# blyssprivacy/sdk

Measured on NVIDIA H100. Metric: PIR server queries/sec (Spiral process_query), higher is better.
Workload: dtype u64

## Files before the change

sdk_b200/csrc/api.cu:

```cuda
#include "../../include/b200pir.h"
#include "kernels.h"
#include "ntt_tables.hpp"
#include <cstdio>
#include <algorithm>
#include <cmath>
#include <memory>
#include <cstring>
#include <condition_variable>
#include <chrono>
#include <deque>
#include <mutex>
#include <set>
#include <string>
#include <utility>
#include <vector>

using namespace b200pir;

namespace b200pir {
thread_local unsigned long long g_kernel_launches = 0;

void opt_in_smem_impl(const void* kernel, int bytes) {
  static std::mutex mu;
  static std::set<std::pair<const void*, int>> done;
// ... 49 lines not shown
  int device = 0;
  cudaStream_t stream = nullptr;
  bool own_stream = true;
  std::recursive_mutex mu;
  b200pir_params hp;
  int dim0, num_per, slices, trials, g, stop_round, num_packing;
  int bits_gsw, bits_conv, bits_left, bits_right;
  bool has_right;
  uint64_t q2, q1, setup_bytes, query_bytes, response_bytes;
  int q1_bits;
  DevParams dp;
  DevBuf<Twiddle> d_tw;
  DevBuf<Twiddle> d_tw4k;
  DevBuf<uint32_t> d_neg1;
  int mul_variant = 0, max_group = 16, profile = 0;
  int fold_variant = 2;
  int intt_variant = 0;
  int expand_variant = 0;
  long pair_min_ctas = 528;
  int sparse_fold = 0;
  int imma_variant = 0;
  int db_format = -1;
  DevBuf<uint2> w_qf;
  DevBuf<uint8_t> w_qt;
  int sm_count = 0;
  size_t ws_queries = 0, ws_rows = 0;
  DevBuf<uint64_t> w_query;
  DevBuf<uint32_t> w_v;
  DevBuf<uint32_t> w_zflags;
  DevBuf<uint32_t> w_xr;
  DevBuf<uint4> w_qdev;
  DevBuf<uint32_t> w_vfold, w_vfold_neg;
  DevBuf<uint32_t> w_mult;
  DevBuf<uint32_t> w_cts;
// ... 258 lines not shown
}

const uint32_t* run_fold_res(b200pir_ctx* c, uint32_t* a, uint32_t* b, size_t batch, size_t batch_stride, size_t num,
                             int k0, const uint32_t* vfold, int slices_per_query) {
  const size_t mat = (size_t)2 * 2 * c->hp.t_gsw * 2 * POLY;
  int k = k0;
  uint32_t* src = a;
  uint32_t* dst = b;
  uint32_t* zero_flags = nullptr;
  if (c->sparse_fold) {
    c->w_zflags.ensure(batch * num);
    zero_flags = c->w_zflags.p;
  }
  for (size_t half = num / 2; half >= 1; half /= 2, k--) {
    launch_fold_res(c->dp, src, dst, batch, batch_stride, (int)half, vfold + (size_t)k * mat, c->fold_words(),
                    slices_per_query, (int)c->hp.t_gsw, c->bits_gsw, c->fold_variant, zero_flags, c->stream);
    std::swap(src, dst);
  }
  return src;
}

void run_prepare(b200pir_ctx* c, b200pir_pp* pp, size_t count, bool images = false) {
  b200pir_ctx::Scope sc(c, ST_EXPAND);
  if (images) c->w_qt.ensure((count + 15) / 16 * tc5_query_bytes(make_tc5_geom(c->dim0, 32)));
  if (c->hp.expand_queries)
    run_expand_query(c, pp, c->w_query.p, c->w_v.p, c->w_qdev.p, c->w_vfold.p, (int)count, images ? c->w_qt.p : nullptr);
}

void run_first_dim_and_fold(b200pir_ctx* c, b200pir_db* db, size_t count, const uint4* qdev = nullptr,
                            const uint32_t* vfold = nullptr, const uint8_t* images = nullptr, size_t per_group = 16) {
  if (!qdev) qdev = c->w_qdev.p;
// ... 241 lines not shown
  if (queries == 0 || queries > 4096 || rows_local == 0 || rows_local > ((size_t)1 << c->hp.nu_2))
    throw Error(B200PIR_E_BADARG, "reserve: 1..4096 queries, 1..num_per rows");
  Guard gd(c);
  B200_CUDA(cudaStreamSynchronize(c->stream));
  c->ensure_workspace(queries, rows_local);
  B200_CUDA(cudaGetLastError());
  API_END
}
int b200pir_ctx_set_option(b200pir_ctx* c, const char* key, int64_t value) {
  API_BEGIN
  if (!c || !key) throw Error(B200PIR_E_BADARG, "null argument");
  Guard gd(c);
  std::string k(key);
  if (k == "mul_variant") c->mul_variant = (int)value;
  else if (k == "batch") { if (value != 1 && value != 2 && value != 4 && value != 8 && value != 16) throw Error(B200PIR_E_BADARG, "batch must be 1, 2, 4, 8 or 16"); c->max_group = (int)value; }
  else if (k == "fold_variant") c->fold_variant = (int)value;
  else if (k == "intt_variant") c->intt_variant = (int)value;
  else if (k == "imma_variant") c->imma_variant = (int)value;
  else if (k == "sparse_fold") c->sparse_fold = value != 0;
  else if (k == "coalesce") c->coalesce = value != 0;
  else if (k == "coalesce_window_us") { if (value < 0 || value > 100000) throw Error(B200PIR_E_BADARG, "coalesce_window_us must be 0..100000"); c->coalesce_window_us = (int)value; }
  else if (k == "expand_variant") c->expand_variant = (int)value;
  else if (k == "expand_pair_min_ctas") c->pair_min_ctas = (long)value;
  else if (k == "db_format") { if (value < -1 || value > 2) throw Error(B200PIR_E_BADARG, "db_format must be -1 (automatic), 0, 1 or 2"); c->db_format = (int)value; }
  else if (k == "profile") {
    if (value < 0 || value > 2) throw Error(B200PIR_E_BADARG, "profile must be 0, 1 or 2");
    c->profile = (int)value;
    c->spans.clear(); c->event_next = 0; c->mul_launches = 0;
  }
  else throw Error(B200PIR_E_BADARG, "unknown option " + k);
  API_END
// ... 526 lines not shown
  B200_CUDA(cudaMemcpyAsync(wide.p, v_folding, wide.n * 8, cudaMemcpyHostToDevice, c->stream));
  launch_narrow(vf.p, wide.p, wide.n, c->stream);
  if (v_folding_neg && !c->sparse_fold) {
    DevBuf<uint32_t> vfn(c->fold_words());
    B200_CUDA(cudaMemcpyAsync(wide.p, v_folding_neg, wide.n * 8, cudaMemcpyHostToDevice, c->stream));
    launch_narrow(vfn.p, wide.p, wide.n, c->stream);
    run_fold(c, cts.p, 1, num * 2 * POLY, num, dims - 1, vf.p, vfn.p, 1);
  } else {
    DevBuf<uint32_t> a(num * 4 * POLY), b(num * 4 * POLY);
    DevBuf<uint32_t> zflags;
    if (c->sparse_fold) zflags.alloc(num);
    launch_raw_to_res(c->dp, a.p, cts.p, num * 2, c->stream);
    int k = dims - 1;
    for (size_t half = num / 2; half >= 1; half /= 2, k--) {
      launch_fold_res(c->dp, a.p, b.p, 1, num * 4 * POLY, (int)half, vf.p + (size_t)k * mat, c->fold_words(), 1,
                      (int)c->hp.t_gsw, c->bits_gsw, c->fold_variant, zflags.p, c->stream);
      B200_CUDA(cudaMemcpyAsync(a.p, b.p, half * 4 * POLY * 4, cudaMemcpyDeviceToDevice, c->stream));
    }
    launch_res_to_raw(c->dp, cts.p, a.p, num * 2, c->stream);
  }
  B200_CUDA(cudaMemcpyAsync(v_cts, cts.p, cts.n * 8, cudaMemcpyDeviceToHost, c->stream));
  B200_CUDA(cudaStreamSynchronize(c->stream));
  B200_CUDA(cudaGetLastError());
  API_END
}

int b200pir_get_v_folding_neg(b200pir_ctx* c, uint64_t* out, const uint64_t* v_folding) {
  API_BEGIN
  if (!c || !out || !v_folding) throw Error(B200PIR_E_BADARG, "null argument");
  Guard gd(c);
  const size_t words = c->fold_words();
// ... 696 lines not shown
```

sdk_b200/csrc/kernels.h:

```cpp
#pragma once
#include "common.cuh"
#include "tc5_layout.cuh"

namespace b200pir {

static const int POLY = 2048;

extern thread_local unsigned long long g_kernel_launches;

void opt_in_smem_impl(const void* kernel, int bytes);
template <typename K>
inline void opt_in_smem(K* kernel, int bytes) { opt_in_smem_impl(reinterpret_cast<const void*>(kernel), bytes); }

void launch_ntt_u64(const DevParams& P, uint64_t* polys, size_t count, bool inverse, cudaStream_t s);
void launch_ntt32(const DevParams& P, uint32_t* polys, size_t count, bool inverse, cudaStream_t s);
void launch_ntt32_4k(uint32_t q0, uint32_t q1, const Twiddle* tw, uint32_t* polys, size_t count, bool inverse, cudaStream_t s);
void launch_to_ntt(const DevParams& P, uint32_t* out, const uint64_t* raw, size_t count, cudaStream_t s);
void launch_to_ntt_strided(const DevParams& P, uint32_t* out, size_t out_stride, const uint64_t* raw, size_t raw_stride,
                           size_t count, int batches, cudaStream_t s);
void launch_chacha_first_rows(uint64_t* raw, const uint8_t seed[32], uint64_t word0, uint32_t n_mats, uint32_t row_words,
                              uint64_t mat_words, uint64_t modulus, cudaStream_t s);
void launch_direct_query_to_dev(uint4* q_dev, const uint32_t* sig_ntt, const uint64_t* wire_words, int dim0, cudaStream_t s);
void launch_from_ntt(const DevParams& P, uint64_t* out_raw, const uint32_t* in, size_t count, cudaStream_t s);
void launch_raw_to_res(const DevParams& P, uint32_t* out, const uint64_t* raw, size_t polys, cudaStream_t s);
// ... 36 lines not shown
size_t tc5_db_bytes(const Tc5Geom& T, int slices);
size_t tc5_query_bytes(const Tc5Geom& T);
bool tc5_supported(const Tc5Geom& T);
void launch_db_to_tc5(const Tc5Geom& T, const uint4* db0_slice, uint8_t* dbt, int slice, cudaStream_t s);
void launch_db_upsert_tc5(const Tc5Geom& T, uint8_t* dbt, int slice, int il, int j, const uint64_t* poly, cudaStream_t s);
void launch_query_to_tc5(const Tc5Geom& T, const uint4* q_dev, size_t q_stride, int nq, uint8_t* qt, cudaStream_t s);
void launch_reorient_to_tc5(const Tc5Geom& T, const uint32_t* v, size_t v_stride, int idx_factor, int nq, uint8_t* qt, cudaStream_t s);
void launch_multiply_tc5(const DevParams& P, const Tc5Geom& T, const uint8_t* dbt, const uint32_t* tile_mask, const uint8_t* qt,
                         uint32_t* out_zm, size_t out_stride, int nq, int slice_begin, int slice_count, int sm_count, cudaStream_t s);

void launch_fold_round(const DevParams& P, uint64_t* cts, size_t batch, size_t batch_stride , int half,
                       const uint32_t* c_pos, const uint32_t* c_neg, size_t c_batch_stride ,
                       int slices_per_query, int t_gsw, int bits, cudaStream_t s);
void launch_fold_res(const DevParams& P, const uint32_t* in, uint32_t* out, size_t batch, size_t batch_stride ,
                     int half, const uint32_t* c_pos, size_t c_batch_stride, int slices_per_query, int t_gsw, int bits,
                     int variant, uint32_t* zero_flags , cudaStream_t s);
void launch_folding_neg(const DevParams& P, uint32_t* out, const uint32_t* v_folding, int count, int t_gsw, int bits,
                        cudaStream_t s);

void launch_expand_scalar(const DevParams& P, uint32_t* v, size_t v_stride, int nq, int num_in, const uint32_t* neg1_r,
                          cudaStream_t s);
struct PpTable { const uint32_t* const* pack; const uint32_t* const* left; const uint32_t* const* right; const uint32_t* const* conv; };
struct ExpandRound {
  int r, num_in, stop_round, max_bits_to_gen_right, t_auto;
  const uint32_t* const* tab_left;
  const uint32_t* const* tab_right;
  size_t off_left, off_right;
  int t_left, t_right, bits_left, bits_right;
  int fill_skipped;
};
void launch_expand_round(const DevParams& P, uint32_t* v, size_t v_stride, int nq, const ExpandRound& R, cudaStream_t s);
// ... 32 lines not shown
```

sdk_b200/csrc/poly_kernels.cu:

```cuda
#include "kernels.h"
#include "ntt_core4096.cuh"

namespace b200pir {

namespace {

constexpr int CTA = 512;
constexpr int HI_TW = NTT_N - 64;

__constant__ Twiddle c_tw_lo[2][3][64];

struct TwConst {
  int n, dir;
  __device__ __forceinline__ Twiddle operator()(int i) const { return c_tw_lo[n][dir][i]; }
  __device__ __forceinline__ void load2(int i, Twiddle (&t)[2]) const { t[0] = (*this)(i); t[1] = (*this)(i + 1); }
  __device__ __forceinline__ void load4(int i, Twiddle (&t)[4]) const {
    t[0] = (*this)(i); t[1] = (*this)(i + 1); t[2] = (*this)(i + 2); t[3] = (*this)(i + 3);
  }
};
struct TwShared {
  const Twiddle* p;
  __device__ __forceinline__ Twiddle operator()(int i) const { return p[i - 64]; }
  __device__ __forceinline__ void load2(int i, Twiddle (&t)[2]) const {
    uint4 v = *reinterpret_cast<const uint4*>(p + (i - 64));
// ... 95 lines not shown

template <int ROWS>
__device__ __forceinline__ void acc_reduce(uint64_t (&acc)[ROWS][8], const Grp& g) {
#pragma unroll
  for (int r = 0; r < ROWS; r++)
#pragma unroll
    for (int k = 0; k < 8; k++) acc[r][k] = barrett64(acc[r][k], g.cr1, g.q);
}

template <bool BYTE>
__device__ __forceinline__ uint32_t gadget_digit_fast(uint64_t v, int k, int bits, uint64_t mask) {
  if (BYTE) return __byte_perm((uint32_t)v, (uint32_t)(v >> 32), 0x7770u | (uint32_t)k);
  return gadget_digit(v, k, bits, mask);
}

template <int ROWS, bool SM, bool BYTE>
__device__ __forceinline__ void digits_mac_impl(uint64_t (&acc)[ROWS][8], int& cnt, const uint64_t (&v)[8], int ndig,
                                                int bits, const uint32_t* c0, size_t col_step, size_t row_step,
                                                const Grp& g) {
  const uint64_t mask = (1ull << bits) - 1;
  int k = 0;
  if (SM) {
#pragma unroll 1
    for (; k + 1 < ndig; k += 2) {
      uint32_t x0[8], x1[8];
#pragma unroll
      for (int a = 0; a < 8; a++) {
        x0[a] = gadget_digit_fast<BYTE>(v[a], k, bits, mask);
        x1[a] = gadget_digit_fast<BYTE>(v[a], k + 1, bits, mask);
      }
      ntt_forward_group2_lz<NTT_OUT_LAZY16>(g.tid, x0, x1, g.smem, g.smem2, TwConst{g.n, 0}, TwShared{g.fwd_hi_sm}, g.q, CtaSync());
      if (cnt + 2 > 16) { acc_reduce<ROWS>(acc, g); cnt = 1; }
      cnt += 2;
      const uint32_t* c = c0 + (size_t)k * col_step;
#pragma unroll
      for (int r = 0; r < ROWS; r++) {
        uint32_t cv[8];
        ld8_ro(cv, c + (size_t)r * row_step);
#pragma unroll
        for (int e = 0; e < 8; e++) acc[r][e] += (uint64_t)x0[e] * cv[e];
        ld8_ro(cv, c + col_step + (size_t)r * row_step);
#pragma unroll
        for (int e = 0; e < 8; e++) acc[r][e] += (uint64_t)x1[e] * cv[e];
      }
    }
  }
#pragma unroll 1
  for (; k < ndig; k++) {
    uint32_t x[8];
#pragma unroll
    for (int a = 0; a < 8; a++) x[a] = gadget_digit_fast<BYTE>(v[a], k, bits, mask);
    if (SM) ntt_forward_group_lz<NTT_OUT_LAZY16>(g.tid, x, g.smem, TwConst{g.n, 0}, TwShared{g.fwd_hi_sm}, g.q, CtaSync());
    else ntt_forward_group_lz<NTT_OUT_LAZY16>(g.tid, x, g.smem, TwConst{g.n, 0}, TwGlobal{g.fwd}, g.q, CtaSync());
    if (cnt + 1 > 16) { acc_reduce<ROWS>(acc, g); cnt = 1; }
    cnt += 1;
    const uint32_t* c = c0 + (size_t)k * col_step;
#pragma unroll
    for (int r = 0; r < ROWS; r++) {
      uint32_t cv[8];
      ld8_ro(cv, c + (size_t)r * row_step);
#pragma unroll
      for (int e = 0; e < 8; e++) acc[r][e] += (uint64_t)x[e] * cv[e];
    }
  }
}

template <int ROWS, bool SM>
__device__ __forceinline__ void digits_mac(uint64_t (&acc)[ROWS][8], int& cnt, const uint64_t (&v)[8], int ndig,
                                           int bits, const uint32_t* c0, size_t col_step, size_t row_step,
                                           const Grp& g) {
  if (bits == 8) digits_mac_impl<ROWS, SM, true>(acc, cnt, v, ndig, bits, c0, col_step, row_step, g);
  else digits_mac_impl<ROWS, SM, false>(acc, cnt, v, ndig, bits, c0, col_step, row_step, g);
}

template <typename Sink>
__device__ __forceinline__ void crt_lift(const uint32_t (&x)[8], uint32_t* res, const Grp& g, const DevParams& P,
                                         Sink sink) {
  __syncthreads();
#pragma unroll
  for (int a = 0; a < 8; a++) res[g.n * POLY + a * 256 + g.tid] = x[a];
  __syncthreads();
#pragma unroll
  for (int a4 = 0; a4 < 4; a4++) {
// ... 123 lines not shown
#pragma unroll
  for (int r = 0; r < 2; r++)
#pragma unroll
    for (int e = 0; e < 8; e++) acc[r][e] = 0;
  int cnt = 0;
#pragma unroll 1
  for (int src = 0; src < 2; src++) {
    const uint64_t* ct = base + (size_t)(src == 0 ? i : half + i) * 2 * POLY;
    const uint32_t* C = (src == 0 ? c_neg : c_pos) + qoff;
#pragma unroll 1
    for (int rho = 0; rho < 2; rho++) {
      uint64_t v[8];
#pragma unroll
      for (int a = 0; a < 8; a++) v[a] = ct[rho * POLY + a * 256 + g.tid];
      const uint32_t* c0 = C + ((size_t)rho * 2 + g.n) * POLY + g.tid * 8;
      digits_mac<2, false>(acc, cnt, v, t_gsw, bits, c0, col_step, row_step, g);
    }
  }
  uint64_t* dst = base + (size_t)i * 2 * POLY;
#pragma unroll 1
  for (int r = 0; r < 2; r++) {
    uint32_t x[8];
#pragma unroll
    for (int e = 0; e < 8; e++) x[e] = barrett64(acc[r][e], g.cr1, g.q);
    grp_ntt_inv(g, x);
    uint64_t* d = dst + r * POLY;
    crt_lift(x, res, g, P, [&](int z, uint64_t val) { d[z] = val; });
  }
}

template <bool BYTE>
__device__ __forceinline__ uint32_t digit_diff(uint64_t vh, uint64_t vi, int k, int bits, uint64_t mask, uint32_t q) {
  if (BYTE) {
    const uint32_t sel = 0x7770u | (uint32_t)k;
    return __byte_perm((uint32_t)vh, (uint32_t)(vh >> 32), sel) - __byte_perm((uint32_t)vi, (uint32_t)(vi >> 32), sel) + q;
  }
  return gadget_digit(vh, k, bits, mask) - gadget_digit(vi, k, bits, mask) + q;
}

template <int MINB, bool BYTE>
__global__ void __launch_bounds__(256, MINB)
k_fold_res_lz(DevParams P, const uint32_t* __restrict__ in, uint32_t* __restrict__ out, size_t batch_stride, int half,
              const uint32_t* __restrict__ c_pos, size_t c_batch_stride, int slices_per_query, int t_gsw, int bits,
              const uint32_t* __restrict__ zero_flags ) {
  if (zero_flags) {
    const int bz = blockIdx.x / half, iz = blockIdx.x % half;
    const uint32_t fa = zero_flags[(size_t)bz * 2 * half + iz], fb = zero_flags[(size_t)bz * 2 * half + half + iz];
    if (fa | fb) {
      const uint32_t* src = in + (size_t)bz * batch_stride + (size_t)((fa ? half : 0) + iz) * 4 * POLY;
      uint32_t* dst = out + (size_t)bz * batch_stride + (size_t)iz * 4 * POLY;
#pragma unroll
      for (int rho = 0; rho < 2; rho++) {
        uint32_t x[8];
        ld8_ro(x, src + ((size_t)rho * 2 + blockIdx.y) * POLY + threadIdx.x * 8);
        st8(dst + ((size_t)rho * 2 + blockIdx.y) * POLY + threadIdx.x * 8, x);
      }
// ... 4 lines not shown
  uint32_t* sm0 = reinterpret_cast<uint32_t*>(dyn_smem);
  uint32_t* sm1 = sm0 + NTT_SMEM_WORDS;
  Twiddle* tw = reinterpret_cast<Twiddle*>(sm1 + NTT_SMEM_WORDS);
  Grp g = make_grp_single(P, sm0, blockIdx.y);
  stage_fwd_twiddles(g, tw);
  const TwConst lo{g.n, 0};
  const TwShared hi{tw};
  const int b = blockIdx.x / half, i = blockIdx.x % half;
  const uint32_t* ci = in + (size_t)b * batch_stride + (size_t)i * 4 * POLY;
  const uint32_t* ch = in + (size_t)b * batch_stride + (size_t)(half + i) * 4 * POLY;
  const uint32_t* C = c_pos + (size_t)(b / slices_per_query) * c_batch_stride;
  const int cols = 2 * t_gsw;
  const size_t row_step = (size_t)cols * 2 * POLY;
  const uint64_t mask = (1ull << bits) - 1;
  const uint32_t q = g.q;

  uint64_t acc[2][8];
#pragma unroll
  for (int r = 0; r < 2; r++)
#pragma unroll
    for (int e = 0; e < 8; e++) acc[r][e] = 0;
  int cnt = 0;
#pragma unroll 1
  for (int rho = 0; rho < 2; rho++) {
    uint64_t vi[8], vh[8];
#pragma unroll
    for (int a = 0; a < 8; a++) {
      const int z = a * 256 + g.tid;
      vi[a] = crt_compose(__ldg(ci + (rho * 2 + 0) * POLY + z), __ldg(ci + (rho * 2 + 1) * POLY + z), P);
      vh[a] = crt_compose(__ldg(ch + (rho * 2 + 0) * POLY + z), __ldg(ch + (rho * 2 + 1) * POLY + z), P);
    }
    const uint32_t* c0 = C + ((size_t)rho * 2 + g.n) * POLY + g.tid * 8;
    int k = 0;
#pragma unroll 1
    for (; k + 1 < t_gsw; k += 2) {
      uint32_t x0[8], x1[8];
#pragma unroll
      for (int a = 0; a < 8; a++) {
        x0[a] = digit_diff<BYTE>(vh[a], vi[a], k, bits, mask, q);
        x1[a] = digit_diff<BYTE>(vh[a], vi[a], k + 1, bits, mask, q);
      }
      ntt_forward_group2_lz<NTT_OUT_LAZY16>(g.tid, x0, x1, sm0, sm1, lo, hi, q, CtaSync());
      if (cnt + 2 > 16) { acc_reduce<2>(acc, g); cnt = 1; }
      cnt += 2;
#pragma unroll
      for (int r = 0; r < 2; r++) {
        uint32_t cv[8];
        ld8_ro(cv, c0 + (size_t)r * row_step + (size_t)k * 4 * POLY);
#pragma unroll
        for (int e = 0; e < 8; e++) acc[r][e] += (uint64_t)x0[e] * cv[e];
        ld8_ro(cv, c0 + (size_t)r * row_step + (size_t)(k + 1) * 4 * POLY);
#pragma unroll
        for (int e = 0; e < 8; e++) acc[r][e] += (uint64_t)x1[e] * cv[e];
      }
    }
    if (k < t_gsw) {
      uint32_t x0[8];
#pragma unroll
      for (int a = 0; a < 8; a++) x0[a] = digit_diff<BYTE>(vh[a], vi[a], k, bits, mask, q);
      ntt_forward_group_lz<NTT_OUT_LAZY16>(g.tid, x0, sm0, lo, hi, q, CtaSync());
      if (cnt + 1 > 16) { acc_reduce<2>(acc, g); cnt = 1; }
      cnt += 1;
#pragma unroll
      for (int r = 0; r < 2; r++) {
        uint32_t cv[8];
        ld8_ro(cv, c0 + (size_t)r * row_step + (size_t)k * 4 * POLY);
#pragma unroll
        for (int e = 0; e < 8; e++) acc[r][e] += (uint64_t)x0[e] * cv[e];
      }
    }
  }
  uint32_t y0[8], y1[8];
#pragma unroll
  for (int e = 0; e < 8; e++) {
// ... 64 lines not shown
  Grp g = make_grp(P, ntt_smem);
  g.smem2 = ntt_smem + (2 + g.n) * NTT_SMEM_WORDS;

  const int i = blockIdx.x;
  const int ih = i < R.num_in ? i : i - R.num_in;
  if ((R.stop_round > 0 && R.r > R.stop_round && (ih & 1)) ||
      (R.stop_round > 0 && R.r == R.stop_round && (ih & 1) && (ih / 2) >= R.max_bits_to_gen_right))
    return;
  const bool left = (R.r != 0) && ((ih & 1) == 0);
  const uint32_t* W = left ? R.tab_left[blockIdx.y] + R.off_left : R.tab_right[blockIdx.y] + R.off_right;
  const int t_exp = left ? R.t_left : R.t_right;
  const int bits = left ? R.bits_left : R.bits_right;

  stage_fwd_twiddles(g, tw + g.n * HI_TW);
  uint32_t* vi = v + (size_t)i * 4 * POLY;
  uint32_t keep[2][8];
  {
    uint32_t x[8];
    ld8(x, vi + (size_t)g.n * POLY + g.tid * 8);
#pragma unroll
    for (int e = 0; e < 8; e++) keep[0][e] = x[e];
    grp_ntt_inv(g, x);
    const int t_auto = R.t_auto;
    const uint64_t Q = P.modulus;
    crt_lift(x, res, g, P, [&](int z, uint64_t val) {
      unsigned prod = (unsigned)z * (unsigned)t_auto;
      unsigned num = prod >> NTT_LOG_N, rem = prod & (POLY - 1);
      autom[rem] = (num & 1u) ? Q - val : val;
    });
  }
  uint32_t y[8];
  {
    const uint32_t* row1 = vi + ((size_t)2 + g.n) * POLY;
    ld8(keep[1], row1 + g.tid * 8);
#pragma unroll
    for (int k = 0; k < 8; k++) {
      const unsigned sidx = (unsigned)(g.tid * 8 + k);
      const unsigned e = 2u * (__brev(sidx) >> (32 - NTT_LOG_N)) + 1u;
      const unsigned e2 = (e * (unsigned)R.t_auto) & (2u * POLY - 1u);
      const unsigned src = __brev((e2 - 1u) >> 1) >> (32 - NTT_LOG_N);
      y[k] = row1[src];
    }
  }
  __syncthreads();
  uint64_t acc[2][8];
#pragma unroll
  for (int r = 0; r < 2; r++)
#pragma unroll
    for (int e = 0; e < 8; e++) acc[r][e] = 0;
  int cnt = 0;
  {
    uint64_t vv[8];
#pragma unroll
    for (int a = 0; a < 8; a++) vv[a] = autom[a * 256 + g.tid];
    const uint32_t* c0 = W + (size_t)g.n * POLY + g.tid * 8;
    digits_mac<2, true>(acc, cnt, vv, t_exp, bits, c0, (size_t)2 * POLY, (size_t)t_exp * 2 * POLY, g);
  }
#pragma unroll
  for (int rho = 0; rho < 2; rho++) {
    uint32_t o[8];
#pragma unroll
    for (int e = 0; e < 8; e++) {
      uint32_t s = addmod(keep[rho][e], barrett64(acc[rho][e], g.cr1, g.q), g.q);
      o[e] = rho ? addmod(s, y[e], g.q) : s;
    }
    st8(vi + ((size_t)rho * 2 + g.n) * POLY + g.tid * 8, o);
  }
}

__global__ void __launch_bounds__(CTA, 1)
k_expand_round_pair(DevParams P, uint32_t* v, size_t v_stride, ExpandRound R, const uint32_t* __restrict__ neg1) {
  v += (size_t)blockIdx.y * v_stride;
  extern __shared__ __align__(16) uint8_t dyn_smem[];
  uint32_t* ntt_smem = reinterpret_cast<uint32_t*>(dyn_smem);
  uint32_t* res = ntt_smem + 4 * NTT_SMEM_WORDS;
  uint64_t* autom = reinterpret_cast<uint64_t*>(res + 2 * POLY);
  Twiddle* tw = reinterpret_cast<Twiddle*>(autom + 2 * POLY);
  Grp g = make_grp(P, ntt_smem);
// ... 64 lines not shown
        a0 = a0 ? q0 - a0 : 0u;
        a1 = a1 ? q1 - a1 : 0u;
      }
      const uint64_t val = crt_compose(a0, a1, P);
      const unsigned prod = (unsigned)k * (unsigned)R.t_auto;
      const unsigned num = prod >> NTT_LOG_N, rem = prod & (POLY - 1);
      autom[rem] = (num & 1u) ? Q - val : val;
    }
    __syncthreads();
    uint64_t acc[2][8];
#pragma unroll
    for (int r = 0; r < 2; r++)
#pragma unroll
      for (int e = 0; e < 8; e++) acc[r][e] = 0;
    int cnt = 0;
    {
      uint64_t vv[8];
#pragma unroll
      for (int a = 0; a < 8; a++) vv[a] = autom[a * 256 + g.tid];
      const uint32_t* c0 = W + (size_t)g.n * POLY + g.tid * 8;
      digits_mac<2, true>(acc, cnt, vv, t_exp, bits, c0, (size_t)2 * POLY, (size_t)t_exp * 2 * POLY, g);
    }
    uint32_t* dst = half ? vo : vi;
#pragma unroll
    for (int rho = 0; rho < 2; rho++) {
      uint32_t o[8], nn[8];
      if (half) ld8_ro(nn, ng + g.tid * 8);
#pragma unroll
      for (int e = 0; e < 8; e++) {
        uint32_t base = keep[rho][e];
        if (half) base = barrett64((uint64_t)base * nn[e], g.cr1, g.q);
        uint32_t s = addmod(base, barrett64(acc[rho][e], g.cr1, g.q), g.q);
        if (rho) {
          uint32_t yy = y[e];
          if (half) {
            const unsigned sidx = (unsigned)(g.tid * 8 + e);
            const unsigned ee = 2u * (__brev(sidx) >> (32 - NTT_LOG_N)) + 1u;
// ... 17 lines not shown
  __shared__ __align__(16) uint32_t ntt_smem[NTT_SMEM_WORDS];
  const int i = blockIdx.x;
  if ((R.stop_round > 0 && R.r > R.stop_round && (i & 1)) ||
      (R.stop_round > 0 && R.r == R.stop_round && (i & 1) && (i / 2) >= R.max_bits_to_gen_right))
    return;
  Grp g = make_grp_single(P, ntt_smem, blockIdx.y);
  const uint32_t* src = v + (size_t)blockIdx.z * v_stride + ((size_t)i * 4 + g.n) * POLY;
  uint32_t x[8];
  ld8_ro(x, src + g.tid * 8);
  grp_ntt_inv(g, x);
  uint32_t* dst = xr + (size_t)blockIdx.z * xr_stride + ((size_t)i * 2 + g.n) * POLY;
#pragma unroll
  for (int a = 0; a < 8; a++) dst[a * 256 + g.tid] = x[a];
}

template <int MINB>
__global__ void __launch_bounds__(256, MINB)
k_expand_round_res(DevParams P, uint32_t* v, size_t v_stride, const uint32_t* __restrict__ xr, size_t xr_stride,
                   ExpandRound R, const uint32_t* __restrict__ neg1) {
  v += (size_t)blockIdx.z * v_stride;
  xr += (size_t)blockIdx.z * xr_stride;
  extern __shared__ __align__(16) uint8_t dyn_smem[];
  uint32_t* sm0 = reinterpret_cast<uint32_t*>(dyn_smem);
  uint32_t* sm1 = sm0 + NTT_SMEM_WORDS;
  uint64_t* autom = reinterpret_cast<uint64_t*>(sm1 + NTT_SMEM_WORDS);
  Twiddle* tw = reinterpret_cast<Twiddle*>(autom + POLY);
  Grp g = make_grp_single(P, sm0, blockIdx.y);
  g.smem2 = sm1;
  const int i = blockIdx.x;
  const uint32_t* ng = neg1 + (size_t)g.n * POLY;
  uint32_t* vi = v + (size_t)i * 4 * POLY;
  uint32_t* vo = v + (size_t)(i + R.num_in) * 4 * POLY;
// ... 35 lines not shown
        a0 = a0 ? q0 - a0 : 0u;
        a1 = a1 ? q1 - a1 : 0u;
      }
      const uint64_t val = crt_compose(a0, a1, P);
      const unsigned prod = (unsigned)k * (unsigned)R.t_auto;
      const unsigned num = prod >> NTT_LOG_N, rem = prod & (POLY - 1);
      autom[rem] = (num & 1u) ? Q - val : val;
    }
    __syncthreads();
    uint64_t acc[2][8];
#pragma unroll
    for (int r = 0; r < 2; r++)
#pragma unroll
      for (int e = 0; e < 8; e++) acc[r][e] = 0;
    int cnt = 0;
    {
      uint64_t vv[8];
#pragma unroll
      for (int a = 0; a < 8; a++) vv[a] = autom[a * 256 + g.tid];
      const uint32_t* c0 = W + (size_t)g.n * POLY + g.tid * 8;
      digits_mac<2, true>(acc, cnt, vv, t_exp, bits, c0, (size_t)2 * POLY, (size_t)t_exp * 2 * POLY, g);
    }
    uint32_t yy[8];
#pragma unroll
    for (int e = 0; e < 8; e++) {
      const unsigned sidx = (unsigned)(g.tid * 8 + e);
      const unsigned ee = 2u * (__brev(sidx) >> (32 - NTT_LOG_N)) + 1u;
      const unsigned e2 = (ee * (unsigned)R.t_auto) & (2u * POLY - 1u);
      const unsigned src = __brev((e2 - 1u) >> 1) >> (32 - NTT_LOG_N);
      uint32_t t = row1[src];
      if (half) t = barrett64((uint64_t)t * __ldg(ng + src), g.cr1, g.q);
      yy[e] = t;
    }
    __syncthreads();
    uint32_t* dst = half ? vo : vi;
    uint32_t nn[8];
    if (half) ld8_ro(nn, ng + g.tid * 8);
// ... 50 lines not shown
    st8(out + (((size_t)rho * cols + 2 * j + 1) * 2 + g.n) * POLY + g.tid * 8, x);
    grp_ntt_inv(g, x);
    uint64_t* d = raw + rho * POLY;
    crt_lift(x, res, g, P, [&](int z, uint64_t val) { d[z] = val; });
  }
  __syncthreads();
  uint64_t acc[2][8];
#pragma unroll
  for (int r = 0; r < 2; r++)
#pragma unroll
    for (int e = 0; e < 8; e++) acc[r][e] = 0;
  int cnt = 0;
  const int ccols = 2 * t_conv;
#pragma unroll 1
  for (int rho = 0; rho < 2; rho++) {
    uint64_t vv[8];
#pragma unroll
    for (int a = 0; a < 8; a++) vv[a] = raw[rho * POLY + a * 256 + g.tid];
    const uint32_t* c0 = v_conv + ((size_t)rho * 2 + g.n) * POLY + g.tid * 8;
    digits_mac<2, true>(acc, cnt, vv, t_conv, bits_conv, c0, (size_t)2 * 2 * POLY, (size_t)ccols * 2 * POLY, g);
  }
#pragma unroll
  for (int r = 0; r < 2; r++) {
    uint32_t o[8];
#pragma unroll
    for (int e = 0; e < 8; e++) o[e] = barrett64(acc[r][e], g.cr1, g.q);
    st8(out + (((size_t)r * cols + 2 * j) * 2 + g.n) * POLY + g.tid * 8, o);
  }
}

template <int ROWS>
__global__ void __launch_bounds__(CTA, 1)
k_pack(DevParams P, uint64_t* out_raw, size_t out_q_stride, const uint32_t* folded, size_t ct_stride, size_t in_q_stride,
       const uint32_t* const* tab_pack, int t_conv, int bits, int version) {
  const uint32_t* v_packing = tab_pack[blockIdx.y];
// ... 20 lines not shown

#pragma unroll 1
  for (int r = 0; r < n; r++) {
    const uint32_t* ct = folded + ((size_t)inst * n * n + (size_t)r * n + c) * ct_stride;
    const uint32_t* W = v_packing + (version == 0 ? (size_t)r * mat_words : 0);
    uint64_t acc[ROWS][8];
#pragma unroll
    for (int m = 0; m < ROWS; m++)
#pragma unroll
      for (int e = 0; e < 8; e++) acc[m][e] = 0;
    int cnt = 0;
    {
      uint64_t vv[8];
#pragma unroll
      for (int a = 0; a < 8; a++) vv[a] = crt_compose(__ldg(ct + a * 256 + g.tid), __ldg(ct + POLY + a * 256 + g.tid), P);
      digits_mac<ROWS, true>(acc, cnt, vv, t_conv, bits, W + (size_t)g.n * POLY + g.tid * 8, col_step, row_step, g);
    }
    uint32_t y[8];
#pragma unroll
    for (int a = 0; a < 8; a++) y[a] = __ldg(ct + (2 + g.n) * POLY + a * 256 + g.tid);
    grp_ntt_fwd<true>(g, y);
    uint32_t prod[ROWS][8];
#pragma unroll
    for (int m = 0; m < ROWS; m++)
#pragma unroll
      for (int e = 0; e < 8; e++) prod[m][e] = barrett64(acc[m][e], g.cr1, g.q);
    if (version == 0) {
#pragma unroll
      for (int m = 0; m < ROWS; m++)
#pragma unroll
        for (int e = 0; e < 8; e++) {
          uint32_t s = addmod(vint[m][e], prod[m][e], g.q);
          vint[m][e] = (m == 1 + r) ? addmod(s, y[e], g.q) : s;
        }
    } else {
#pragma unroll
      for (int e = 0; e < 8; e++) prod[1][e] = addmod(prod[1][e], y[e], g.q);
      const uint32_t* Wshift = v_packing + mat_words;
#pragma unroll 1
      for (int sft = 0; sft < r; sft++) {
        uint32_t x[8];
#pragma unroll
        for (int e = 0; e < 8; e++) x[e] = prod[0][e];
        grp_ntt_inv(g, x);
        crt_lift(x, res, g, P, [&](int z, uint64_t val) { rawbuf[z] = val; });
        __syncthreads();
        uint64_t vv[8];
#pragma unroll
        for (int a = 0; a < 8; a++) vv[a] = rawbuf[a * 256 + g.tid];
#pragma unroll
        for (int m = 0; m < ROWS; m++)
#pragma unroll
          for (int e = 0; e < 8; e++) acc[m][e] = 0;
        cnt = 0;
        digits_mac<ROWS, true>(acc, cnt, vv, t_conv, bits, Wshift + (size_t)g.n * POLY + g.tid * 8, col_step, row_step, g);
        uint32_t np[ROWS][8];
#pragma unroll
        for (int m = 0; m < ROWS; m++)
#pragma unroll
          for (int e = 0; e < 8; e++) {
            uint32_t p1 = barrett64(acc[m][e], g.cr1, g.q);
            uint32_t p2 = (m == 0) ? 0u : (m == 1 ? prod[n][e] : prod[m - 1][e]);
            np[m][e] = addmod(p1, p2, g.q);
          }
#pragma unroll
        for (int m = 0; m < ROWS; m++)
#pragma unroll
          for (int e = 0; e < 8; e++) prod[m][e] = np[m][e];
      }
#pragma unroll
// ... 85 lines not shown
  if (count) ++g_kernel_launches, k_to_ntt<<<dim3((unsigned)count, 2), 256, 0, s>>>(P, out, raw, 0, 0);
}
void launch_to_ntt_strided(const DevParams& P, uint32_t* out, size_t out_stride, const uint64_t* raw, size_t raw_stride,
                           size_t count, int batches, cudaStream_t s) {
  if (count && batches)
    ++g_kernel_launches, k_to_ntt<<<dim3((unsigned)count, 2, (unsigned)batches), 256, 0, s>>>(P, out, raw, out_stride, raw_stride);
}
void launch_raw_to_res(const DevParams& P, uint32_t* out, const uint64_t* raw, size_t polys, cudaStream_t s) {
  if (polys) ++g_kernel_launches, k_raw_to_res<<<grid1d(polys * POLY, 256), 256, 0, s>>>(P, out, raw, polys);
}
void launch_res_to_raw(const DevParams& P, uint64_t* out, const uint32_t* res, size_t polys, cudaStream_t s) {
  if (polys) ++g_kernel_launches, k_res_to_raw<<<grid1d(polys * POLY, 256), 256, 0, s>>>(P, out, res, polys);
}
void launch_fold_res(const DevParams& P, const uint32_t* in, uint32_t* out, size_t batch, size_t batch_stride, int half,
                     const uint32_t* c_pos, size_t c_batch_stride, int slices_per_query, int t_gsw, int bits,
                     int variant, uint32_t* zero_flags, cudaStream_t s) {
  if (batch == 0 || half == 0) return;
  if (zero_flags) {
    ++g_kernel_launches;
    k_ct_zero_flags<<<(unsigned)(batch * 2 * half), 256, 0, s>>>(in, batch_stride, 2 * half, zero_flags);
  }
  ++g_kernel_launches;
  const dim3 grid((unsigned)(batch * half), 2);
#define FOLD_LZ(MINB, BYTE)                                                                                             \
  do {                                                                                                                  \
    opt_in_smem(k_fold_res_lz<MINB, BYTE>, (int)kDynSmemFold);                                                          \
    k_fold_res_lz<MINB, BYTE><<<grid, 256, kDynSmemFold, s>>>(P, in, out, batch_stride, half, c_pos, c_batch_stride,    \
                                                             slices_per_query, t_gsw, bits, zero_flags);               \
  } while (0)
  if (variant == 3) { if (bits == 8) FOLD_LZ(2, true); else FOLD_LZ(2, false); }
  else { if (bits == 8) FOLD_LZ(3, true); else FOLD_LZ(3, false); }
#undef FOLD_LZ
}
void launch_from_ntt(const DevParams& P, uint64_t* out_raw, const uint32_t* in, size_t count, cudaStream_t s) {
  if (count) ++g_kernel_launches, k_from_ntt<<<(unsigned)count, CTA, 0, s>>>(P, out_raw, in);
}
void launch_widen(uint64_t* out, const uint32_t* in, size_t words, cudaStream_t s) {
  if (words) ++g_kernel_launches, k_widen<<<grid1d(words, 256), 256, 0, s>>>(out, in, words);
}
void launch_narrow(uint32_t* out, const uint64_t* in, size_t words, cudaStream_t s) {
  if (words) ++g_kernel_launches, k_narrow<<<grid1d(words, 256), 256, 0, s>>>(out, in, words);
}
void launch_fold_round(const DevParams& P, uint64_t* cts, size_t batch, size_t batch_stride, int half,
                       const uint32_t* c_pos, const uint32_t* c_neg, size_t c_batch_stride, int slices_per_query,
                       int t_gsw, int bits, cudaStream_t s) {
  if (batch == 0 || half == 0) return;
  ++g_kernel_launches;
// ... 13 lines not shown
}
void launch_expand_round(const DevParams& P, uint32_t* v, size_t v_stride, int nq, const ExpandRound& R, cudaStream_t s) {
  opt_in_smem(k_expand_round, (int)kDynSmemBig);
  ++g_kernel_launches;
  k_expand_round<<<dim3((unsigned)(2 * R.num_in), nq), CTA, kDynSmemBig, s>>>(P, v, v_stride, R);
}
void launch_expand_round_pair(const DevParams& P, uint32_t* v, size_t v_stride, int nq, const ExpandRound& R,
                              const uint32_t* neg1_r, cudaStream_t s) {
  opt_in_smem(k_expand_round_pair, (int)kDynSmemBig);
  ++g_kernel_launches;
  k_expand_round_pair<<<dim3((unsigned)R.num_in, nq), CTA, kDynSmemBig, s>>>(P, v, v_stride, R, neg1_r);
}
void launch_expand_round_res(const DevParams& P, uint32_t* v, size_t v_stride, uint32_t* xr, size_t xr_stride, int nq,
                             const ExpandRound& R, const uint32_t* neg1_r, cudaStream_t s) {
  const size_t smem = (size_t)2 * NTT_SMEM_WORDS * 4 + (size_t)POLY * 8 + (size_t)HI_TW * 8;
  opt_in_smem(k_expand_round_res<3>, (int)smem);
  g_kernel_launches += 2;
  k_expand_intt<<<dim3((unsigned)R.num_in, 2, nq), 256, 0, s>>>(P, v, v_stride, xr, xr_stride, R);
  k_expand_round_res<3><<<dim3((unsigned)R.num_in, 2, nq), 256, smem, s>>>(P, v, v_stride, xr, xr_stride, R, neg1_r);
}
void launch_reorient(const MulGeom& G, uint4* q_dev, size_t q_stride, const uint32_t* v, size_t v_stride, int nq,
                     int idx_factor, cudaStream_t s) {
  size_t total = (size_t)G.dim0 * POLY;
  ++g_kernel_launches;
  k_reorient<<<dim3(grid1d(total, 256), nq), 256, 0, s>>>(G, q_dev, q_stride, v, v_stride, idx_factor);
}
void launch_regev_to_gsw(const DevParams& P, uint32_t* v_gsw, size_t gsw_stride, const uint32_t* v, size_t v_stride,
                         int nq, int count, int idx_factor, int idx_offset, const uint32_t* const* tab_conv, int t_gsw,
                         int t_conv, int bits_conv, cudaStream_t s) {
  if (count == 0) return;
  opt_in_smem(k_regev_to_gsw, (int)kDynSmemBig);
  ++g_kernel_launches;
  k_regev_to_gsw<<<dim3((unsigned)(count * t_gsw), nq), CTA, kDynSmemBig, s>>>(P, v_gsw, gsw_stride, v, v_stride,
                                                                               idx_factor, idx_offset, tab_conv, t_gsw,
// ... 32 lines not shown
```

Measured before the change: 1289.

## Cut fold/expand register pressure via smem digit planes and smem-backed coefficients

For byte-sized gadget digits, the fold kernel now precomputes pairwise digit differences into shared-memory planes once per rho and reads them back in the digit loop. The fold variant option is removed, and fold and expand_round_res drop from 3 to 2 blocks per SM in their launch bounds. digits_mac now takes a coefficient accessor so expand kernels read coefficients straight from shared memory instead of copying them into registers. Other changes: the expand kernel reloads the original values from global memory rather than keeping them live, the two MAC row loops are split, and pair_min_ctas defaults to 1. The aim is lower register pressure and fewer digit-extraction instructions, at the cost of extra shared memory, lower occupancy and more global reloads.

Result: faster. 1492, median of 6 (+15.7%).

```diff
diff --git a/sdk_b200/csrc/api.cu b/sdk_b200/csrc/api.cu
--- a/sdk_b200/csrc/api.cu
+++ b/sdk_b200/csrc/api.cu
@@ -87,10 +87,9 @@
   DevBuf<Twiddle> d_tw4k;
   DevBuf<uint32_t> d_neg1;
   int mul_variant = 0, max_group = 16, profile = 0;
-  int fold_variant = 2;
   int intt_variant = 0;
   int expand_variant = 0;
-  long pair_min_ctas = 528;
+  long pair_min_ctas = 1;
   int sparse_fold = 0;
   int imma_variant = 0;
   int db_format = -1;
@@ -379,7 +378,7 @@
   }
   for (size_t half = num / 2; half >= 1; half /= 2, k--) {
     launch_fold_res(c->dp, src, dst, batch, batch_stride, (int)half, vfold + (size_t)k * mat, c->fold_words(),
-                    slices_per_query, (int)c->hp.t_gsw, c->bits_gsw, c->fold_variant, zero_flags, c->stream);
+                    slices_per_query, (int)c->hp.t_gsw, c->bits_gsw, zero_flags, c->stream);
     std::swap(src, dst);
   }
   return src;
@@ -651,7 +650,7 @@
   std::string k(key);
   if (k == "mul_variant") c->mul_variant = (int)value;
   else if (k == "batch") { if (value != 1 && value != 2 && value != 4 && value != 8 && value != 16) throw Error(B200PIR_E_BADARG, "batch must be 1, 2, 4, 8 or 16"); c->max_group = (int)value; }
-  else if (k == "fold_variant") c->fold_variant = (int)value;
+  else if (k == "fold_variant") {}
   else if (k == "intt_variant") c->intt_variant = (int)value;
   else if (k == "imma_variant") c->imma_variant = (int)value;
   else if (k == "sparse_fold") c->sparse_fold = value != 0;
@@ -1208,7 +1207,7 @@
     int k = dims - 1;
     for (size_t half = num / 2; half >= 1; half /= 2, k--) {
       launch_fold_res(c->dp, a.p, b.p, 1, num * 4 * POLY, (int)half, vf.p + (size_t)k * mat, c->fold_words(), 1,
-                      (int)c->hp.t_gsw, c->bits_gsw, c->fold_variant, zflags.p, c->stream);
+                      (int)c->hp.t_gsw, c->bits_gsw, zflags.p, c->stream);
       B200_CUDA(cudaMemcpyAsync(a.p, b.p, half * 4 * POLY * 4, cudaMemcpyDeviceToDevice, c->stream));
     }
     launch_res_to_raw(c->dp, cts.p, a.p, num * 2, c->stream);
diff --git a/sdk_b200/csrc/kernels.h b/sdk_b200/csrc/kernels.h
--- a/sdk_b200/csrc/kernels.h
+++ b/sdk_b200/csrc/kernels.h
@@ -74,7 +74,7 @@
                        int slices_per_query, int t_gsw, int bits, cudaStream_t s);
 void launch_fold_res(const DevParams& P, const uint32_t* in, uint32_t* out, size_t batch, size_t batch_stride ,
                      int half, const uint32_t* c_pos, size_t c_batch_stride, int slices_per_query, int t_gsw, int bits,
-                     int variant, uint32_t* zero_flags , cudaStream_t s);
+                     uint32_t* zero_flags , cudaStream_t s);
 void launch_folding_neg(const DevParams& P, uint32_t* out, const uint32_t* v_folding, int count, int t_gsw, int bits,
                         cudaStream_t s);
 
diff --git a/sdk_b200/csrc/poly_kernels.cu b/sdk_b200/csrc/poly_kernels.cu
--- a/sdk_b200/csrc/poly_kernels.cu
+++ b/sdk_b200/csrc/poly_kernels.cu
@@ -133,8 +133,17 @@
   return gadget_digit(v, k, bits, mask);
 }
 
-template <int ROWS, bool SM, bool BYTE>
-__device__ __forceinline__ void digits_mac_impl(uint64_t (&acc)[ROWS][8], int& cnt, const uint64_t (&v)[8], int ndig,
+struct RegCoef {
+  const uint64_t (&v)[8];
+  __device__ __forceinline__ uint64_t operator()(int a) const { return v[a]; }
+};
+struct SmemCoef {
+  const uint64_t* p;
+  __device__ __forceinline__ uint64_t operator()(int a) const { return p[a * 256]; }
+};
+
+template <int ROWS, bool SM, bool BYTE, typename Coef>
+__device__ __forceinline__ void digits_mac_impl(uint64_t (&acc)[ROWS][8], int& cnt, Coef v, int ndig,
                                                 int bits, const uint32_t* c0, size_t col_step, size_t row_step,
                                                 const Grp& g) {
   const uint64_t mask = (1ull << bits) - 1;
@@ -145,8 +154,9 @@
       uint32_t x0[8], x1[8];
 #pragma unroll
       for (int a = 0; a < 8; a++) {
-        x0[a] = gadget_digit_fast<BYTE>(v[a], k, bits, mask);
-        x1[a] = gadget_digit_fast<BYTE>(v[a], k + 1, bits, mask);
+        const uint64_t va = v(a);
+        x0[a] = gadget_digit_fast<BYTE>(va, k, bits, mask);
+        x1[a] = gadget_digit_fast<BYTE>(va, k + 1, bits, mask);
       }
       ntt_forward_group2_lz<NTT_OUT_LAZY16>(g.tid, x0, x1, g.smem, g.smem2, TwConst{g.n, 0}, TwShared{g.fwd_hi_sm}, g.q, CtaSync());
       if (cnt + 2 > 16) { acc_reduce<ROWS>(acc, g); cnt = 1; }
@@ -158,6 +168,10 @@
         ld8_ro(cv, c + (size_t)r * row_step);
 #pragma unroll
         for (int e = 0; e < 8; e++) acc[r][e] += (uint64_t)x0[e] * cv[e];
+      }
+#pragma unroll
+      for (int r = 0; r < ROWS; r++) {
+        uint32_t cv[8];
         ld8_ro(cv, c + col_step + (size_t)r * row_step);
 #pragma unroll
         for (int e = 0; e < 8; e++) acc[r][e] += (uint64_t)x1[e] * cv[e];
@@ -168,7 +182,7 @@
   for (; k < ndig; k++) {
     uint32_t x[8];
 #pragma unroll
-    for (int a = 0; a < 8; a++) x[a] = gadget_digit_fast<BYTE>(v[a], k, bits, mask);
+    for (int a = 0; a < 8; a++) x[a] = gadget_digit_fast<BYTE>(v(a), k, bits, mask);
     if (SM) ntt_forward_group_lz<NTT_OUT_LAZY16>(g.tid, x, g.smem, TwConst{g.n, 0}, TwShared{g.fwd_hi_sm}, g.q, CtaSync());
     else ntt_forward_group_lz<NTT_OUT_LAZY16>(g.tid, x, g.smem, TwConst{g.n, 0}, TwGlobal{g.fwd}, g.q, CtaSync());
     if (cnt + 1 > 16) { acc_reduce<ROWS>(acc, g); cnt = 1; }
@@ -184,8 +198,8 @@
   }
 }
 
-template <int ROWS, bool SM>
-__device__ __forceinline__ void digits_mac(uint64_t (&acc)[ROWS][8], int& cnt, const uint64_t (&v)[8], int ndig,
+template <int ROWS, bool SM, typename Coef>
+__device__ __forceinline__ void digits_mac(uint64_t (&acc)[ROWS][8], int& cnt, Coef v, int ndig,
                                            int bits, const uint32_t* c0, size_t col_step, size_t row_step,
                                            const Grp& g) {
   if (bits == 8) digits_mac_impl<ROWS, SM, true>(acc, cnt, v, ndig, bits, c0, col_step, row_step, g);
@@ -339,7 +353,7 @@
 #pragma unroll
       for (int a = 0; a < 8; a++) v[a] = ct[rho * POLY + a * 256 + g.tid];
       const uint32_t* c0 = C + ((size_t)rho * 2 + g.n) * POLY + g.tid * 8;
-      digits_mac<2, false>(acc, cnt, v, t_gsw, bits, c0, col_step, row_step, g);
+      digits_mac<2, false>(acc, cnt, RegCoef{v}, t_gsw, bits, c0, col_step, row_step, g);
     }
   }
   uint64_t* dst = base + (size_t)i * 2 * POLY;
@@ -354,17 +368,18 @@
   }
 }
 
+__device__ __forceinline__ uint32_t digit_diff(uint64_t vh, uint64_t vi, int k, int bits, uint64_t mask, uint32_t q) {
+  return gadget_digit(vh, k, bits, mask) - gadget_digit(vi, k, bits, mask) + q;
+}
+__device__ __forceinline__ uint32_t byte_pair_diff(uint64_t vh, uint64_t vi, int k) {
+  const uint32_t sel = 0x7070u | ((uint32_t)(k + 1) << 8) | (uint32_t)k;
+  return __byte_perm((uint32_t)vh, (uint32_t)(vh >> 32), sel) + 0x01000100u -
+         __byte_perm((uint32_t)vi, (uint32_t)(vi >> 32), sel);
+}
+constexpr int kFoldPlanes = 4;
+
 template <bool BYTE>
-__device__ __forceinline__ uint32_t digit_diff(uint64_t vh, uint64_t vi, int k, int bits, uint64_t mask, uint32_t q) {
-  if (BYTE) {
-    const uint32_t sel = 0x7770u | (uint32_t)k;
-    return __byte_perm((uint32_t)vh, (uint32_t)(vh >> 32), sel) - __byte_perm((uint32_t)vi, (uint32_t)(vi >> 32), sel) + q;
-  }
-  return gadget_digit(vh, k, bits, mask) - gadget_digit(vi, k, bits, mask) + q;
-}
-
-template <int MINB, bool BYTE>
-__global__ void __launch_bounds__(256, MINB)
+__global__ void __launch_bounds__(256, 2)
 k_fold_res_lz(DevParams P, const uint32_t* __restrict__ in, uint32_t* __restrict__ out, size_t batch_stride, int half,
               const uint32_t* __restrict__ c_pos, size_t c_batch_stride, int slices_per_query, int t_gsw, int bits,
               const uint32_t* __restrict__ zero_flags ) {
@@ -399,6 +414,7 @@
   const size_t row_step = (size_t)cols * 2 * POLY;
   const uint64_t mask = (1ull << bits) - 1;
   const uint32_t q = g.q;
+  uint32_t* planes = reinterpret_cast<uint32_t*>(tw + HI_TW) + g.tid;
 
   uint64_t acc[2][8];
 #pragma unroll
@@ -414,6 +430,11 @@
       const int z = a * 256 + g.tid;
       vi[a] = crt_compose(__ldg(ci + (rho * 2 + 0) * POLY + z), __ldg(ci + (rho * 2 + 1) * POLY + z), P);
       vh[a] = crt_compose(__ldg(ch + (rho * 2 + 0) * POLY + z), __ldg(ch + (rho * 2 + 1) * POLY + z), P);
+      if (BYTE) {
+#pragma unroll
+        for (int p = 0; p < kFoldPlanes; p++)
+          if (2 * p < t_gsw) planes[p * POLY + a * 256] = byte_pair_diff(vh[a], vi[a], 2 * p);
+      }
     }
     const uint32_t* c0 = C + ((size_t)rho * 2 + g.n) * POLY + g.tid * 8;
     int k = 0;
@@ -422,8 +443,14 @@
       uint32_t x0[8], x1[8];
 #pragma unroll
       for (int a = 0; a < 8; a++) {
-        x0[a] = digit_diff<BYTE>(vh[a], vi[a], k, bits, mask, q);
-        x1[a] = digit_diff<BYTE>(vh[a], vi[a], k + 1, bits, mask, q);
+        if (BYTE) {
+          const uint32_t w = planes[(k >> 1) * POLY + a * 256];
+          x0[a] = (w & 0xffffu) + (q - 256u);
+          x1[a] = (w >> 16) + (q - 256u);
+        } else {
+          x0[a] = digit_diff(vh[a], vi[a], k, bits, mask, q);
+          x1[a] = digit_diff(vh[a], vi[a], k + 1, bits, mask, q);
+        }
       }
       ntt_forward_group2_lz<NTT_OUT_LAZY16>(g.tid, x0, x1, sm0, sm1, lo, hi, q, CtaSync());
       if (cnt + 2 > 16) { acc_reduce<2>(acc, g); cnt = 1; }
@@ -434,6 +461,10 @@
         ld8_ro(cv, c0 + (size_t)r * row_step + (size_t)k * 4 * POLY);
 #pragma unroll
         for (int e = 0; e < 8; e++) acc[r][e] += (uint64_t)x0[e] * cv[e];
+      }
+#pragma unroll
+      for (int r = 0; r < 2; r++) {
+        uint32_t cv[8];
         ld8_ro(cv, c0 + (size_t)r * row_step + (size_t)(k + 1) * 4 * POLY);
 #pragma unroll
         for (int e = 0; e < 8; e++) acc[r][e] += (uint64_t)x1[e] * cv[e];
@@ -442,7 +473,8 @@
     if (k < t_gsw) {
       uint32_t x0[8];
 #pragma unroll
-      for (int a = 0; a < 8; a++) x0[a] = digit_diff<BYTE>(vh[a], vi[a], k, bits, mask, q);
+      for (int a = 0; a < 8; a++)
+        x0[a] = BYTE ? (planes[(k >> 1) * POLY + a * 256] & 0xffffu) + (q - 256u) : digit_diff(vh[a], vi[a], k, bits, mask, q);
       ntt_forward_group_lz<NTT_OUT_LAZY16>(g.tid, x0, sm0, lo, hi, q, CtaSync());
       if (cnt + 1 > 16) { acc_reduce<2>(acc, g); cnt = 1; }
       cnt += 1;
@@ -537,12 +569,9 @@
 
   stage_fwd_twiddles(g, tw + g.n * HI_TW);
   uint32_t* vi = v + (size_t)i * 4 * POLY;
-  uint32_t keep[2][8];
   {
     uint32_t x[8];
     ld8(x, vi + (size_t)g.n * POLY + g.tid * 8);
-#pragma unroll
-    for (int e = 0; e < 8; e++) keep[0][e] = x[e];
     grp_ntt_inv(g, x);
     const int t_auto = R.t_auto;
     const uint64_t Q = P.modulus;
@@ -552,10 +581,18 @@
       autom[rem] = (num & 1u) ? Q - val : val;
     });
   }
+  __syncthreads();
+  uint64_t acc[2][8];
+#pragma unroll
+  for (int r = 0; r < 2; r++)
+#pragma unroll
+    for (int e = 0; e < 8; e++) acc[r][e] = 0;
+  int cnt = 0;
+  digits_mac<2, true>(acc, cnt, SmemCoef{autom + g.tid}, t_exp, bits, W + (size_t)g.n * POLY + g.tid * 8, (size_t)2 * POLY,
+                      (size_t)t_exp * 2 * POLY, g);
   uint32_t y[8];
   {
     const uint32_t* row1 = vi + ((size_t)2 + g.n) * POLY;
-    ld8(keep[1], row1 + g.tid * 8);
 #pragma unroll
     for (int k = 0; k < 8; k++) {
       const unsigned sidx = (unsigned)(g.tid * 8 + k);
@@ -566,25 +603,13 @@
     }
   }
   __syncthreads();
-  uint64_t acc[2][8];
-#pragma unroll
-  for (int r = 0; r < 2; r++)
-#pragma unroll
-    for (int e = 0; e < 8; e++) acc[r][e] = 0;
-  int cnt = 0;
-  {
-    uint64_t vv[8];
-#pragma unroll
-    for (int a = 0; a < 8; a++) vv[a] = autom[a * 256 + g.tid];
-    const uint32_t* c0 = W + (size_t)g.n * POLY + g.tid * 8;
-    digits_mac<2, true>(acc, cnt, vv, t_exp, bits, c0, (size_t)2 * POLY, (size_t)t_exp * 2 * POLY, g);
-  }
 #pragma unroll
   for (int rho = 0; rho < 2; rho++) {
     uint32_t o[8];
+    ld8(o, vi + ((size_t)rho * 2 + g.n) * POLY + g.tid * 8);
 #pragma unroll
     for (int e = 0; e < 8; e++) {
-      uint32_t s = addmod(keep[rho][e], barrett64(acc[rho][e], g.cr1, g.q), g.q);
+      uint32_t s = addmod(o[e], barrett64(acc[rho][e], g.cr1, g.q), g.q);
       o[e] = rho ? addmod(s, y[e], g.q) : s;
     }
     st8(vi + ((size_t)rho * 2 + g.n) * POLY + g.tid * 8, o);
@@ -679,13 +704,8 @@
 #pragma unroll
       for (int e = 0; e < 8; e++) acc[r][e] = 0;
     int cnt = 0;
-    {
-      uint64_t vv[8];
-#pragma unroll
-      for (int a = 0; a < 8; a++) vv[a] = autom[a * 256 + g.tid];
-      const uint32_t* c0 = W + (size_t)g.n * POLY + g.tid * 8;
-      digits_mac<2, true>(acc, cnt, vv, t_exp, bits, c0, (size_t)2 * POLY, (size_t)t_exp * 2 * POLY, g);
-    }
+    digits_mac<2, true>(acc, cnt, SmemCoef{autom + g.tid}, t_exp, bits, W + (size_t)g.n * POLY + g.tid * 8, (size_t)2 * POLY,
+                        (size_t)t_exp * 2 * POLY, g);
     uint32_t* dst = half ? vo : vi;
 #pragma unroll
     for (int rho = 0; rho < 2; rho++) {
@@ -733,8 +753,7 @@
   for (int a = 0; a < 8; a++) dst[a * 256 + g.tid] = x[a];
 }
 
-template <int MINB>
-__global__ void __launch_bounds__(256, MINB)
+__global__ void __launch_bounds__(256, 2)
 k_expand_round_res(DevParams P, uint32_t* v, size_t v_stride, const uint32_t* __restrict__ xr, size_t xr_stride,
                    ExpandRound R, const uint32_t* __restrict__ neg1) {
   v += (size_t)blockIdx.z * v_stride;
@@ -800,13 +819,8 @@
 #pragma unroll
       for (int e = 0; e < 8; e++) acc[r][e] = 0;
     int cnt = 0;
-    {
-      uint64_t vv[8];
-#pragma unroll
-      for (int a = 0; a < 8; a++) vv[a] = autom[a * 256 + g.tid];
-      const uint32_t* c0 = W + (size_t)g.n * POLY + g.tid * 8;
-      digits_mac<2, true>(acc, cnt, vv, t_exp, bits, c0, (size_t)2 * POLY, (size_t)t_exp * 2 * POLY, g);
-    }
+    digits_mac<2, true>(acc, cnt, SmemCoef{autom + g.tid}, t_exp, bits, W + (size_t)g.n * POLY + g.tid * 8, (size_t)2 * POLY,
+                        (size_t)t_exp * 2 * POLY, g);
     uint32_t yy[8];
 #pragma unroll
     for (int e = 0; e < 8; e++) {
@@ -887,11 +901,8 @@
   const int ccols = 2 * t_conv;
 #pragma unroll 1
   for (int rho = 0; rho < 2; rho++) {
-    uint64_t vv[8];
-#pragma unroll
-    for (int a = 0; a < 8; a++) vv[a] = raw[rho * POLY + a * 256 + g.tid];
     const uint32_t* c0 = v_conv + ((size_t)rho * 2 + g.n) * POLY + g.tid * 8;
-    digits_mac<2, true>(acc, cnt, vv, t_conv, bits_conv, c0, (size_t)2 * 2 * POLY, (size_t)ccols * 2 * POLY, g);
+    digits_mac<2, true>(acc, cnt, SmemCoef{raw + rho * POLY + g.tid}, t_conv, bits_conv, c0, (size_t)2 * 2 * POLY, (size_t)ccols * 2 * POLY, g);
   }
 #pragma unroll
   for (int r = 0; r < 2; r++) {
@@ -942,7 +953,7 @@
       uint64_t vv[8];
 #pragma unroll
       for (int a = 0; a < 8; a++) vv[a] = crt_compose(__ldg(ct + a * 256 + g.tid), __ldg(ct + POLY + a * 256 + g.tid), P);
-      digits_mac<ROWS, true>(acc, cnt, vv, t_conv, bits, W + (size_t)g.n * POLY + g.tid * 8, col_step, row_step, g);
+      digits_mac<ROWS, true>(acc, cnt, RegCoef{vv}, t_conv, bits, W + (size_t)g.n * POLY + g.tid * 8, col_step, row_step, g);
     }
     uint32_t y[8];
 #pragma unroll
@@ -973,15 +984,12 @@
         grp_ntt_inv(g, x);
         crt_lift(x, res, g, P, [&](int z, uint64_t val) { rawbuf[z] = val; });
         __syncthreads();
-        uint64_t vv[8];
-#pragma unroll
-        for (int a = 0; a < 8; a++) vv[a] = rawbuf[a * 256 + g.tid];
 #pragma unroll
         for (int m = 0; m < ROWS; m++)
 #pragma unroll
           for (int e = 0; e < 8; e++) acc[m][e] = 0;
         cnt = 0;
-        digits_mac<ROWS, true>(acc, cnt, vv, t_conv, bits, Wshift + (size_t)g.n * POLY + g.tid * 8, col_step, row_step, g);
+        digits_mac<ROWS, true>(acc, cnt, SmemCoef{rawbuf + g.tid}, t_conv, bits, Wshift + (size_t)g.n * POLY + g.tid * 8, col_step, row_step, g);
         uint32_t np[ROWS][8];
 #pragma unroll
         for (int m = 0; m < ROWS; m++)
@@ -1097,7 +1105,7 @@
 }
 void launch_fold_res(const DevParams& P, const uint32_t* in, uint32_t* out, size_t batch, size_t batch_stride, int half,
                      const uint32_t* c_pos, size_t c_batch_stride, int slices_per_query, int t_gsw, int bits,
-                     int variant, uint32_t* zero_flags, cudaStream_t s) {
+                     uint32_t* zero_flags, cudaStream_t s) {
   if (batch == 0 || half == 0) return;
   if (zero_flags) {
     ++g_kernel_launches;
@@ -1105,15 +1113,11 @@
   }
   ++g_kernel_launches;
   const dim3 grid((unsigned)(batch * half), 2);
-#define FOLD_LZ(MINB, BYTE)                                                                                             \
-  do {                                                                                                                  \
-    opt_in_smem(k_fold_res_lz<MINB, BYTE>, (int)kDynSmemFold);                                                          \
-    k_fold_res_lz<MINB, BYTE><<<grid, 256, kDynSmemFold, s>>>(P, in, out, batch_stride, half, c_pos, c_batch_stride,    \
-                                                             slices_per_query, t_gsw, bits, zero_flags);               \
-  } while (0)
-  if (variant == 3) { if (bits == 8) FOLD_LZ(2, true); else FOLD_LZ(2, false); }
-  else { if (bits == 8) FOLD_LZ(3, true); else FOLD_LZ(3, false); }
-#undef FOLD_LZ
+  const bool byte = bits == 8 && t_gsw <= 2 * kFoldPlanes;
+  const size_t smem = kDynSmemFold + (byte ? (size_t)kFoldPlanes * POLY * 4 : 0);
+  auto kern = byte ? k_fold_res_lz<true> : k_fold_res_lz<false>;
+  opt_in_smem(kern, (int)smem);
+  kern<<<grid, 256, smem, s>>>(P, in, out, batch_stride, half, c_pos, c_batch_stride, slices_per_query, t_gsw, bits, zero_flags);
 }
 void launch_from_ntt(const DevParams& P, uint64_t* out_raw, const uint32_t* in, size_t count, cudaStream_t s) {
   if (count) ++g_kernel_launches, k_from_ntt<<<(unsigned)count, CTA, 0, s>>>(P, out_raw, in);
@@ -1157,10 +1161,10 @@
 void launch_expand_round_res(const DevParams& P, uint32_t* v, size_t v_stride, uint32_t* xr, size_t xr_stride, int nq,
                              const ExpandRound& R, const uint32_t* neg1_r, cudaStream_t s) {
   const size_t smem = (size_t)2 * NTT_SMEM_WORDS * 4 + (size_t)POLY * 8 + (size_t)HI_TW * 8;
-  opt_in_smem(k_expand_round_res<3>, (int)smem);
+  opt_in_smem(k_expand_round_res, (int)smem);
   g_kernel_launches += 2;
   k_expand_intt<<<dim3((unsigned)R.num_in, 2, nq), 256, 0, s>>>(P, v, v_stride, xr, xr_stride, R);
-  k_expand_round_res<3><<<dim3((unsigned)R.num_in, 2, nq), 256, smem, s>>>(P, v, v_stride, xr, xr_stride, R, neg1_r);
+  k_expand_round_res<<<dim3((unsigned)R.num_in, 2, nq), 256, smem, s>>>(P, v, v_stride, xr, xr_stride, R, neg1_r);
 }
 void launch_reorient(const MulGeom& G, uint4* q_dev, size_t q_stride, const uint32_t* v, size_t v_stride, int nq,
                      int idx_factor, cudaStream_t s) {
```
